# tanm-sys/forge-ec

Hardware: AMD Instinct MI355X
Metric: secp256k1-var scalar-muls/sec (batched, bit-exact vs CPU oracle on the parity sample) (higher is better)
Workload: dtype u32

## Files before the change

### forge_ec_amd/build.py

```python
import hashlib
import os
import subprocess
import sys

HERE = os.path.dirname(os.path.abspath(__file__))
SRC_DIR = os.path.join(HERE, "csrc")
OBJ_DIR = os.path.join(SRC_DIR, "_obj")
SO = os.path.join(HERE, "libfecgpu.so")
STAMP = SO + ".sha256"
SOURCES = ["fecgpu.hip", "canon.hip", "kernels_p256.hip", "kernels_ed.hip", "kernels_secp.hip", "kernels_codec.hip", "kernels_ecdsa.hip", "kernels_x25519.hip"]
HEADERS = ["coop.hpp", "sched_lf.hpp", "limbs.hpp", "staging.hpp", "host_ctx.hpp", "secp256k1.hpp", "p256.hpp", "ed25519.hpp", "curve25519.hpp",
           "canon_curves.hpp", "canon_kernels.hpp", "field_asm.inc", "kernels.hpp", "cu_split.hpp", os.path.join("..", "..", "include", "fecgpu.h"),
           os.path.join("..", "..", "include", "fecgpu_canon.h")]
FLAGS = ["--offload-arch=gfx950", "-O3", "-std=c++17", "-fPIC"]


def source_hash():
    h = hashlib.sha256(" ".join(FLAGS).encode())
    for rel in SOURCES + HEADERS:
        with open(os.path.join(SRC_DIR, rel), "rb") as f:
            h.update(rel.encode() + b"\0" + f.read())
    return h.hexdigest()


def up_to_date():
    try:
        return os.path.exists(SO) and open(STAMP).read().strip() == source_hash()
    except OSError:
        return False


DECLARATION_ONLY = ("kernels.hpp",)


def tu_closure_hash(src, kernel_code_only=False):
    import re
    seen, todo = [], [src]
    while todo:
        rel = todo.pop()
        if rel in seen or not os.path.exists(os.path.join(SRC_DIR, rel)) or (kernel_code_only and rel in DECLARATION_ONLY):
            continue
        seen.append(rel)
        with open(os.path.join(SRC_DIR, rel), "r") as f:
            todo += re.findall(r'^\s*#\s*include\s+"([^"/]+)"', f.read(), flags=re.M)
    h = hashlib.sha256(" ".join(FLAGS).encode())
    for rel in sorted(seen):
        with open(os.path.join(SRC_DIR, rel), "rb") as f:
            h.update(rel.encode() + b"\0" + f.read())
    return h.hexdigest()


WORKLOAD_TU = {"secp256k1-var": "kernels_secp.hip", "secp256k1-fixed": "kernels_secp.hip",
               "p256-var": "kernels_p256.hip", "p256-fixed": "kernels_p256.hip",
               "ed25519-var": "kernels_ed.hip", "ed25519-fixed": "kernels_ed.hip", "secp256k1-double": "kernels_secp.hip"}


def _tu_hash(src):
    return tu_closure_hash(src)


def build(force=False, verbose=False):
    if not force and up_to_date():
        return SO
    hipcc = os.environ.get("HIPCC", "/opt/rocm/bin/hipcc")
# ... 39 lines not shown
```

### forge_ec_amd/csrc/field_asm.inc

```
#pragma once

#define FEC_SECP_MUL_ASM \
      "v_mov_b32_e32 v165, 0\n\t" \
      "v_mov_b32_e32 v163, 0\n\t" \
      "v_mad_u64_u32 v[132:133], vcc, %10, %18, 0\n\t" \
      "v_mov_b32_e32 v162, v133\n\t" \
      "v_mad_u64_u32 v[134:135], vcc, %10, %19, v[162:163]\n\t" \
      "v_mad_u64_u32 v[134:135], vcc, %11, %18, v[134:135]\n\t" \
      "v_addc_co_u32_e32 v163, vcc, 0, v163, vcc\n\t" \
      "v_mul_lo_u32 v133, v132, %26\n\t" \
      "v_mov_b32_e32 v162, v135\n\t" \
      "v_mad_u64_u32 v[166:167], %9, v133, %27, 0\n\t" \
      "v_add_co_u32_e64 v164, %8, v167, v133\n\t" \
      "v_mad_u64_u32 v[136:137], vcc, %10, %20, v[162:163]\n\t" \
      "v_addc_co_u32_e64 v163, vcc, 0, 0, vcc\n\t" \
      "v_sub_u32_e32 v135, v134, v164\n\t" \
      "v_mad_u64_u32 v[136:137], vcc, %11, %19, v[136:137]\n\t" \
      "v_addc_co_u32_e32 v163, vcc, 0, v163, vcc\n\t" \
      "v_mul_lo_u32 v135, v135, %26\n\t" \
      "v_mad_u64_u32 v[136:137], vcc, %12, %18, v[136:137]\n\t" \
      "v_addc_co_u32_e32 v163, vcc, 0, v163, vcc\n\t" \
      "v_mad_u64_u32 v[166:167], %9, v135, %27, v[164:165]\n\t" \
      "v_mov_b32_e32 v162, v137\n\t" \
      "v_addc_co_u32_e64 v164, %8, v167, v135, %8\n\t" \
// ... 1235 lines not shown
      "v_alignbit_b32 v126, v126, v124, 31\n\t" \
      "v_lshlrev_b32_e32 v124, 1, v124\n\t" \
      "v_add_co_u32_e32 v124, vcc, v124, v153\n\t" \
      "v_addc_co_u32_e32 v126, vcc, v126, v154, vcc\n\t" \
      "v_addc_co_u32_e32 v128, vcc, v128, v155, vcc\n\t" \
      "v_addc_co_u32_e32 v130, vcc, v130, v156, vcc\n\t" \
      "v_addc_co_u32_e32 v132, vcc, v132, v157, vcc\n\t" \
      "v_addc_co_u32_e32 v134, vcc, v134, v158, vcc\n\t" \
      "v_addc_co_u32_e32 v136, vcc, v136, v159, vcc\n\t" \
      "v_addc_co_u32_e32 v138, vcc, v138, v160, vcc\n\t" \
      "v_addc_co_u32_e32 v140, vcc, v140, v161, vcc\n\t" \
      "v_addc_co_u32_e32 v142, vcc, v142, v162, vcc\n\t" \
      "v_addc_co_u32_e32 v144, vcc, v144, v163, vcc\n\t" \
      "v_addc_co_u32_e32 v146, vcc, v146, v164, vcc\n\t" \
      "v_addc_co_u32_e32 v148, vcc, v148, v165, vcc\n\t" \
      "v_addc_co_u32_e32 v149, vcc, v149, v166, vcc\n\t" \
      "v_addc_co_u32_e32 v151, vcc, v151, v167, vcc\n\t" \
      "v_mov_b32_e32 v153, 0\n\t" \
      "v_mov_b32_e32 v125, 0\n\t" \
      "v_mov_b32_e32 v127, 0\n\t" \
      "v_mov_b32_e32 v129, 0\n\t" \
      "v_mov_b32_e32 v131, 0\n\t" \
      "v_mov_b32_e32 v133, 0\n\t" \
      "v_mov_b32_e32 v135, 0\n\t" \
      "v_mov_b32_e32 v137, 0\n\t" \
      "v_mad_u64_u32 v[152:153], %8, v138, 38, v[152:153]\n\t" \
      "v_mad_u64_u32 v[124:125], %8, v140, 38, v[124:125]\n\t" \
      "v_mad_u64_u32 v[126:127], %8, v142, 38, v[126:127]\n\t" \
      "v_mad_u64_u32 v[128:129], %8, v144, 38, v[128:129]\n\t" \
      "v_mad_u64_u32 v[130:131], %8, v146, 38, v[130:131]\n\t" \
      "v_mad_u64_u32 v[132:133], %8, v148, 38, v[132:133]\n\t" \
      "v_mad_u64_u32 v[134:135], %8, v149, 38, v[134:135]\n\t" \
      "v_mad_u64_u32 v[136:137], %8, v151, 38, v[136:137]\n\t" \
      "v_add_co_u32_e32 %1, vcc, v124, v153\n\t" \
      "v_addc_co_u32_e32 %2, vcc, v126, v125, vcc\n\t" \
      "v_addc_co_u32_e32 %3, vcc, v128, v127, vcc\n\t" \
      "v_addc_co_u32_e32 %4, vcc, v130, v129, vcc\n\t" \
      "v_addc_co_u32_e32 %5, vcc, v132, v131, vcc\n\t" \
      "v_addc_co_u32_e32 %6, vcc, v134, v133, vcc\n\t" \
      "v_addc_co_u32_e32 %7, vcc, v136, v135, vcc\n\t" \
      "v_addc_co_u32_e32 v150, vcc, 0, v137, vcc\n\t" \
      "v_mul_u32_u24_e32 v150, 19, v150\n\t" \
      "v_add_co_u32_e32 %0, vcc, v152, v150\n\t" \
      "s_mov_b64 %9, vcc\n\t" \
      "v_lshrrev_b32_e32 v150, 31, %7\n\t" \
      "v_and_b32_e32 %7, 0x7fffffff, %7\n\t" \
      "v_mul_u32_u24_e32 v150, 19, v150\n\t" \
      "v_add_co_u32_e32 %0, vcc, %0, v150\n\t" \
      "s_or_b64 %9, %9, vcc\n\t" \
      "v_cmp_eq_u32_e32 vcc, 0x7fffffff, %7\n\t" \
      "s_or_b64 %9, %9, vcc"

#define FEC_ED_SQR_CLOBBERS "vcc", "v122", "v123", "v124", "v125", "v126", "v127", "v128", "v129", "v130", "v131", "v132", "v133", "v134", "v135", "v136", "v137", "v138", "v139", "v140", "v141", "v142", "v143", "v144", "v145", "v146", "v147", "v148", "v149", "v150", "v151", "v152", "v153", "v154", "v155", "v156", "v157", "v158", "v159", "v160", "v161", "v162", "v163", "v164", "v165", "v166", "v167"
```

### forge_ec_amd/csrc/kernels_secp.hip

```cpp
#include <hip/hip_runtime.h>

#include "../../include/fecgpu.h"
#include "secp256k1.hpp"
#include "staging.hpp"
#include "kernels.hpp"

namespace fecgpu {

namespace {

FEC_DEV secp::pt ld3(const u32* l, int stride) {
  secp::pt p;
  FEC_UNROLL for (int i = 0; i < 8; ++i) {
    p.x.w[i] = l[i * stride];
    p.y.w[i] = l[(8 + i) * stride];
    p.z.w[i] = l[(16 + i) * stride];
  }
  return p;
}
FEC_DEV void st3(u32* l, int stride, const secp::pt& p) {
  FEC_UNROLL for (int i = 0; i < 8; ++i) {
    l[i * stride] = p.x.w[i];
    l[(8 + i) * stride] = p.y.w[i];
    l[(16 + i) * stride] = p.z.w[i];
  }
}

FEC_DEV fe ldc(const u32* l, int c) {
  fe a;
  FEC_UNROLL for (int i = 0; i < 8; ++i) a.w[i] = l[(8 * c + i) * TPB];
  return a;
}

FEC_DEV secp::pt padd_slots(const u32* lp, const u32* lq, lmask& need_double) {
  using namespace secp;
  fe z1s, z1c, z2s, z2c;
  lmask maybe;
  {
    const fe z1 = ldc(lp, 2);
    maybe = lanes_where(z1.w[0] == 0u);
    z1s = sqr(z1);
    z1c = mul(z1s, z1);
  }
  __builtin_amdgcn_sched_barrier(0);
  {
    const fe z2 = ldc(lq, 2);
    maybe |= lanes_where(z2.w[0] == 0u);
    z2s = sqr(z2);
    z2c = mul(z2s, z2);
  }
  __builtin_amdgcn_sched_barrier(0);
  const fe u1 = mul(ldc(lp, 0), z2s);
  const fe u2 = mul(ldc(lq, 0), z1s);
  __builtin_amdgcn_sched_barrier(0);
  const fe s1 = mul(ldc(lp, 1), z2c);
  const fe s2 = mul(ldc(lq, 1), z1c);
// ... 28 lines not shown

template <int MODE>
__global__ __launch_bounds__(TPB, 3) void k_secp_mul(const u32* __restrict__ scalars,
                                                  const u32* __restrict__ points,
                                                  u32* __restrict__ out, size_t n,
                                                  const u32* __restrict__ prefix, int wbits) {
  __shared__ u32 lds[48 * TPB];
  const int valid = block_valid(n);
  const size_t first = (size_t)blockIdx.x * TPB;
  const int e = threadIdx.x;
  if (MODE == 0) stage_in<24>(lds, points + first * 24, valid);
  __syncthreads();
  if (e < valid) {
    const size_t g = first + e;
    const u32* kg = scalars + g * 8;
    lmask early = 0;
    u32* const slot0 = lds + e;
    int i0 = 0, i1 = 256;
    if (MODE != 3) {
      u32 any = 0;
      FEC_UNROLL for (int i = 0; i < 8; ++i) any |= kg[i];
      early = lanes_where(any == 0);
    }
    if (MODE == 2) early |= secp::is_identity(ld3(points, 1));
    if (MODE == 2 || MODE == 3) {
      const u32 idx = MODE == 3 ? (u32)(g >> 1) : __builtin_bswap32(kg[0]) >> (32 - wbits);
      const uint4* row = reinterpret_cast<const uint4*>(prefix + (size_t)idx * 48);
      FEC_UNROLL for (int q = 0; q < 12; ++q) {
        const uint4 x = row[q];
        slot0[(4 * q + 0) * TPB] = x.x;
        slot0[(4 * q + 1) * TPB] = x.y;
        slot0[(4 * q + 2) * TPB] = x.z;
        slot0[(4 * q + 3) * TPB] = x.w;
      }
      i0 = MODE == 3 ? 0 : wbits;
      if (MODE == 3) i1 = 1;
    } else {
      const secp::pt r1 = MODE != 0 ? ld3(points, 1) : ld3(lds + e, TPB);
      early |= secp::is_identity(r1);
      st3(slot0, TPB, secp::identity());
      st3(slot0 + 24 * TPB, TPB, r1);
    }
    u32 kword = MODE == 3 ? 0u : kg[i0 >> 5];
#pragma unroll 1
    for (int i = i0; i < i1; ++i) {
      u32 b;
      if (MODE == 3) {
        b = (u32)g & 1u;
      } else {
        if ((i & 31) == 0) kword = kg[i >> 5];
        const int sh = (((i >> 3) & 3) << 3) + 7 - (i & 7);
        b = (kword >> sh) & 1u;
      }
      lmask nd;
      secp::pt s = padd_slots(slot0, slot0 + 24 * TPB, nd);
      if (__builtin_expect(nd != 0, 0)) {
        secp::pt d0 = secp::pdouble(ld3(slot0, TPB));
        s = secp::pt_select(s, d0, nd);
      }
      u32* const slot_d = slot0 + b * (24u * TPB);
      u32* const slot_s = slot0 + (b ^ 1u) * (24u * TPB);
      const secp::pt din = ld3(slot_d, TPB);
      st3(slot_s, TPB, s);
      st3(slot_d, TPB, secp::pdouble(din));
    }
    if (MODE != 3) {
      const secp::pt r0 = secp::pt_select(ld3(slot0, TPB), secp::identity(), early);
      st3(slot0, TPB, r0);
    }
  }
  __syncthreads();
  if (MODE == 3) stage_out<48>(out + first * 48, lds, valid);
  else stage_out<24>(out + first * 24, lds, valid);
}

void secp_launch_mul(const SchedEnv& env, bool fixed, const u32* scalars, const u32* points, u32* out, size_t n, hipStream_t s) {
  const unsigned grid = (unsigned)((n + TPB - 1) / TPB);
  const int w = (int)env.gen_prefix_bits[FEC_SECP256K1];
  if (fixed && w > 0 && points == env.gen[FEC_SECP256K1] && env.gen_prefix[FEC_SECP256K1] != nullptr)
    hipLaunchKernelGGL((k_secp_mul<2>), dim3(grid), dim3(TPB), 0, s, scalars, points, out, n, env.gen_prefix[FEC_SECP256K1], w);
  else if (fixed) hipLaunchKernelGGL((k_secp_mul<1>), dim3(grid), dim3(TPB), 0, s, scalars, points, out, n, (const u32*)nullptr, 0);
  else hipLaunchKernelGGL((k_secp_mul<0>), dim3(grid), dim3(TPB), 0, s, scalars, points, out, n, (const u32*)nullptr, 0);
}

void secp_prefix_level_launch(const u32* parent, u32* child, size_t child_entries, hipStream_t s) {
  hipLaunchKernelGGL((k_secp_mul<3>), dim3((unsigned)((child_entries + TPB - 1) / TPB)), dim3(TPB), 0, s, (const u32*)nullptr,
                     (const u32*)nullptr, child, child_entries, parent, 0);
}

}
```

Baseline: 36.38 million.

## Add lazy-reduction secp ladder step with exact fallback on rare carries

New measurement: 37.14 million (median of 6 runs). 2.1% higher.

```diff
diff --git a/forge_ec_amd/build.py b/forge_ec_amd/build.py
--- a/forge_ec_amd/build.py
+++ b/forge_ec_amd/build.py
@@ -9,7 +9,7 @@
 SO = os.path.join(HERE, "libfecgpu.so")
 STAMP = SO + ".sha256"
 SOURCES = ["fecgpu.hip", "canon.hip", "kernels_p256.hip", "kernels_ed.hip", "kernels_secp.hip", "kernels_codec.hip", "kernels_ecdsa.hip", "kernels_x25519.hip"]
-HEADERS = ["coop.hpp", "sched_lf.hpp", "limbs.hpp", "staging.hpp", "host_ctx.hpp", "secp256k1.hpp", "p256.hpp", "ed25519.hpp", "curve25519.hpp",
+HEADERS = ["coop.hpp", "sched_lf.hpp", "limbs.hpp", "staging.hpp", "host_ctx.hpp", "secp256k1.hpp", "secp_step.hpp", "p256.hpp", "ed25519.hpp", "curve25519.hpp",
            "canon_curves.hpp", "canon_kernels.hpp", "field_asm.inc", "kernels.hpp", "cu_split.hpp", os.path.join("..", "..", "include", "fecgpu.h"),
            os.path.join("..", "..", "include", "fecgpu_canon.h")]
 FLAGS = ["--offload-arch=gfx950", "-O3", "-std=c++17", "-fPIC"]
diff --git a/forge_ec_amd/csrc/field_asm.inc b/forge_ec_amd/csrc/field_asm.inc
--- a/forge_ec_amd/csrc/field_asm.inc
+++ b/forge_ec_amd/csrc/field_asm.inc
@@ -1311,3 +1311,543 @@
       "s_or_b64 %9, %9, vcc"
 
 #define FEC_ED_SQR_CLOBBERS "vcc", "v122", "v123", "v124", "v125", "v126", "v127", "v128", "v129", "v130", "v131", "v132", "v133", "v134", "v135", "v136", "v137", "v138", "v139", "v140", "v141", "v142", "v143", "v144", "v145", "v146", "v147", "v148", "v149", "v150", "v151", "v152", "v153", "v154", "v155", "v156", "v157", "v158", "v159", "v160", "v161", "v162", "v163", "v164", "v165", "v166", "v167"
+
+
+#define FEC_SECP_MUL_ACC_ASM \
+      "v_mov_b32_e32 v165, 0\n\t" \
+      "v_mov_b32_e32 v163, 0\n\t" \
+      "v_mad_u64_u32 v[132:133], vcc, %11, %19, 0\n\t" \
+      "v_mov_b32_e32 v162, v133\n\t" \
+      "v_mad_u64_u32 v[134:135], vcc, %11, %20, v[162:163]\n\t" \
+      "v_mad_u64_u32 v[134:135], vcc, %12, %19, v[134:135]\n\t" \
+      "v_addc_co_u32_e32 v163, vcc, 0, v163, vcc\n\t" \
+      "v_mul_lo_u32 v133, v132, %27\n\t" \
+      "v_mov_b32_e32 v162, v135\n\t" \
+      "v_mad_u64_u32 v[166:167], %9, v133, %28, 0\n\t" \
+      "v_add_co_u32_e64 v164, %8, v167, v133\n\t" \
+      "v_mad_u64_u32 v[136:137], vcc, %11, %21, v[162:163]\n\t" \
+      "v_addc_co_u32_e64 v163, vcc, 0, 0, vcc\n\t" \
+      "v_sub_u32_e32 v135, v134, v164\n\t" \
+      "v_mad_u64_u32 v[136:137], vcc, %12, %20, v[136:137]\n\t" \
+      "v_addc_co_u32_e32 v163, vcc, 0, v163, vcc\n\t" \
+      "v_mul_lo_u32 v135, v135, %27\n\t" \
+      "v_mad_u64_u32 v[136:137], vcc, %13, %19, v[136:137]\n\t" \
+      "v_addc_co_u32_e32 v163, vcc, 0, v163, vcc\n\t" \
+      "v_mad_u64_u32 v[166:167], %9, v135, %28, v[164:165]\n\t" \
+      "v_mov_b32_e32 v162, v137\n\t" \
+      "v_addc_co_u32_e64 v164, %8, v167, v135, %8\n\t" \
+      "v_mad_u64_u32 v[138:139], vcc, %11, %22, v[162:163]\n\t" \
+      "v_addc_co_u32_e64 v163, vcc, 0, 0, vcc\n\t" \
+      "v_sub_u32_e32 v137, v136, v164\n\t" \
+      "v_mad_u64_u32 v[138:139], vcc, %12, %21, v[138:139]\n\t" \
+      "v_addc_co_u32_e32 v163, vcc, 0, v163, vcc\n\t" \
+      "v_mul_lo_u32 v137, v137, %27\n\t" \
+      "v_mad_u64_u32 v[138:139], vcc, %13, %20, v[138:139]\n\t" \
+      "v_addc_co_u32_e32 v163, vcc, 0, v163, vcc\n\t" \
+      "v_mad_u64_u32 v[166:167], %9, v137, %28, v[164:165]\n\t" \
+      "v_mad_u64_u32 v[138:139], vcc, %14, %19, v[138:139]\n\t" \
+      "v_addc_co_u32_e32 v163, vcc, 0, v163, vcc\n\t" \
+      "v_addc_co_u32_e64 v164, %8, v167, v137, %8\n\t" \
+      "v_mov_b32_e32 v162, v139\n\t" \
+      "v_mad_u64_u32 v[140:141], vcc, %11, %23, v[162:163]\n\t" \
+      "v_addc_co_u32_e64 v163, vcc, 0, 0, vcc\n\t" \
+      "v_sub_u32_e32 v139, v138, v164\n\t" \
+      "v_mad_u64_u32 v[140:141], vcc, %12, %22, v[140:141]\n\t" \
+      "v_addc_co_u32_e32 v163, vcc, 0, v163, vcc\n\t" \
+      "v_mul_lo_u32 v139, v139, %27\n\t" \
+      "v_mad_u64_u32 v[140:141], vcc, %13, %21, v[140:141]\n\t" \
+      "v_addc_co_u32_e32 v163, vcc, 0, v163, vcc\n\t" \
+      "v_mad_u64_u32 v[166:167], %9, v139, %28, v[164:165]\n\t" \
+      "v_mad_u64_u32 v[140:141], vcc, %14, %20, v[140:141]\n\t" \
+      "v_addc_co_u32_e32 v163, vcc, 0, v163, vcc\n\t" \
+      "v_addc_co_u32_e64 v164, %8, v167, v139, %8\n\t" \
+      "v_mad_u64_u32 v[140:141], vcc, %15, %19, v[140:141]\n\t" \
+      "v_addc_co_u32_e32 v163, vcc, 0, v163, vcc\n\t" \
+      "v_mov_b32_e32 v162, v141\n\t" \
+      "v_mad_u64_u32 v[142:143], vcc, %11, %24, v[162:163]\n\t" \
+      "v_addc_co_u32_e64 v163, vcc, 0, 0, vcc\n\t" \
+      "v_sub_u32_e32 v141, v140, v164\n\t" \
+      "v_mad_u64_u32 v[142:143], vcc, %12, %23, v[142:143]\n\t" \
+      "v_addc_co_u32_e32 v163, vcc, 0, v163, vcc\n\t" \
+      "v_mul_lo_u32 v141, v141, %27\n\t" \
+      "v_mad_u64_u32 v[142:143], vcc, %13, %22, v[142:143]\n\t" \
+      "v_addc_co_u32_e32 v163, vcc, 0, v163, vcc\n\t" \
+      "v_mad_u64_u32 v[166:167], %9, v141, %28, v[164:165]\n\t" \
+      "v_mad_u64_u32 v[142:143], vcc, %14, %21, v[142:143]\n\t" \
+      "v_addc_co_u32_e32 v163, vcc, 0, v163, vcc\n\t" \
+      "v_addc_co_u32_e64 v164, %8, v167, v141, %8\n\t" \
+      "v_mad_u64_u32 v[142:143], vcc, %15, %20, v[142:143]\n\t" \
+      "v_addc_co_u32_e32 v163, vcc, 0, v163, vcc\n\t" \
+      "v_mad_u64_u32 v[142:143], vcc, %16, %19, v[142:143]\n\t" \
+      "v_addc_co_u32_e32 v163, vcc, 0, v163, vcc\n\t" \
+      "v_mov_b32_e32 v162, v143\n\t" \
+      "v_mad_u64_u32 v[144:145], vcc, %11, %25, v[162:163]\n\t" \
+      "v_addc_co_u32_e64 v163, vcc, 0, 0, vcc\n\t" \
+      "v_sub_u32_e32 v143, v142, v164\n\t" \
+      "v_mad_u64_u32 v[144:145], vcc, %12, %24, v[144:145]\n\t" \
+      "v_addc_co_u32_e32 v163, vcc, 0, v163, vcc\n\t" \
+      "v_mul_lo_u32 v143, v143, %27\n\t" \
+      "v_mad_u64_u32 v[144:145], vcc, %13, %23, v[144:145]\n\t" \
+      "v_addc_co_u32_e32 v163, vcc, 0, v163, vcc\n\t" \
+      "v_mad_u64_u32 v[166:167], %9, v143, %28, v[164:165]\n\t" \
+      "v_mad_u64_u32 v[144:145], vcc, %14, %22, v[144:145]\n\t" \
+      "v_addc_co_u32_e32 v163, vcc, 0, v163, vcc\n\t" \
+      "v_addc_co_u32_e64 v164, %8, v167, v143, %8\n\t" \
+      "v_mad_u64_u32 v[144:145], vcc, %15, %21, v[144:145]\n\t" \
+      "v_addc_co_u32_e32 v163, vcc, 0, v163, vcc\n\t" \
+      "v_mad_u64_u32 v[144:145], vcc, %16, %20, v[144:145]\n\t" \
+      "v_addc_co_u32_e32 v163, vcc, 0, v163, vcc\n\t" \
+      "v_mad_u64_u32 v[144:145], vcc, %17, %19, v[144:145]\n\t" \
+      "v_addc_co_u32_e32 v163, vcc, 0, v163, vcc\n\t" \
+      "v_mov_b32_e32 v162, v145\n\t" \
+      "v_mad_u64_u32 v[146:147], vcc, %11, %26, v[162:163]\n\t" \
+      "v_addc_co_u32_e64 v163, vcc, 0, 0, vcc\n\t" \
+      "v_sub_u32_e32 v145, v144, v164\n\t" \
+      "v_mad_u64_u32 v[146:147], vcc, %12, %25, v[146:147]\n\t" \
+      "v_addc_co_u32_e32 v163, vcc, 0, v163, vcc\n\t" \
+      "v_mul_lo_u32 v145, v145, %27\n\t" \
+      "v_mad_u64_u32 v[146:147], vcc, %13, %24, v[146:147]\n\t" \
+      "v_addc_co_u32_e32 v163, vcc, 0, v163, vcc\n\t" \
+      "v_mad_u64_u32 v[166:167], %9, v145, %28, v[164:165]\n\t" \
+      "v_mad_u64_u32 v[146:147], vcc, %14, %23, v[146:147]\n\t" \
+      "v_addc_co_u32_e32 v163, vcc, 0, v163, vcc\n\t" \
+      "v_addc_co_u32_e64 v164, %8, v167, v145, %8\n\t" \
+      "v_mad_u64_u32 v[146:147], vcc, %15, %22, v[146:147]\n\t" \
+      "v_addc_co_u32_e32 v163, vcc, 0, v163, vcc\n\t" \
+      "v_mad_u64_u32 v[146:147], vcc, %16, %21, v[146:147]\n\t" \
+      "v_addc_co_u32_e32 v163, vcc, 0, v163, vcc\n\t" \
+      "v_mad_u64_u32 v[146:147], vcc, %17, %20, v[146:147]\n\t" \
+      "v_addc_co_u32_e32 v163, vcc, 0, v163, vcc\n\t" \
+      "v_mad_u64_u32 v[146:147], vcc, %18, %19, v[146:147]\n\t" \
+      "v_addc_co_u32_e32 v163, vcc, 0, v163, vcc\n\t" \
+      "v_mov_b32_e32 v162, v147\n\t" \
+      "v_mad_u64_u32 v[148:149], vcc, %12, %26, v[162:163]\n\t" \
+      "v_addc_co_u32_e64 v163, vcc, 0, 0, vcc\n\t" \
+      "v_sub_u32_e32 v147, v146, v164\n\t" \
+      "v_mad_u64_u32 v[148:149], vcc, %13, %25, v[148:149]\n\t" \
+      "v_addc_co_u32_e32 v163, vcc, 0, v163, vcc\n\t" \
+      "v_mul_lo_u32 v147, v147, %27\n\t" \
+      "v_mad_u64_u32 v[148:149], vcc, %14, %24, v[148:149]\n\t" \
+      "v_addc_co_u32_e32 v163, vcc, 0, v163, vcc\n\t" \
+      "v_mad_u64_u32 v[166:167], %9, v147, %28, v[164:165]\n\t" \
+      "v_mad_u64_u32 v[148:149], vcc, %15, %23, v[148:149]\n\t" \
+      "v_addc_co_u32_e32 v163, vcc, 0, v163, vcc\n\t" \
+      "v_addc_co_u32_e64 v164, %8, v167, v147, %8\n\t" \
+      "v_mad_u64_u32 v[148:149], vcc, %16, %22, v[148:149]\n\t" \
+      "v_addc_co_u32_e32 v163, vcc, 0, v163, vcc\n\t" \
+      "v_mad_u64_u32 v[148:149], vcc, %17, %21, v[148:149]\n\t" \
+      "v_addc_co_u32_e32 v163, vcc, 0, v163, vcc\n\t" \
+      "v_mad_u64_u32 v[148:149], vcc, %18, %20, v[148:149]\n\t" \
+      "v_addc_co_u32_e32 v163, vcc, 0, v163, vcc\n\t" \
+      "v_mov_b32_e32 v162, v149\n\t" \
+      "v_mad_u64_u32 v[150:151], vcc, %13, %26, v[162:163]\n\t" \
+      "v_addc_co_u32_e64 v163, vcc, 0, 0, vcc\n\t" \
+      "v_mad_u64_u32 v[150:151], vcc, %14, %25, v[150:151]\n\t" \
+      "v_addc_co_u32_e32 v163, vcc, 0, v163, vcc\n\t" \
+      "v_mad_u64_u32 v[150:151], vcc, %15, %24, v[150:151]\n\t" \
+      "v_addc_co_u32_e32 v163, vcc, 0, v163, vcc\n\t" \
+      "v_mad_u64_u32 v[150:151], vcc, %16, %23, v[150:151]\n\t" \
+      "v_addc_co_u32_e32 v163, vcc, 0, v163, vcc\n\t" \
+      "v_mad_u64_u32 v[150:151], vcc, %17, %22, v[150:151]\n\t" \
+      "v_addc_co_u32_e32 v163, vcc, 0, v163, vcc\n\t" \
+      "v_mad_u64_u32 v[150:151], vcc, %18, %21, v[150:151]\n\t" \
+      "v_addc_co_u32_e32 v163, vcc, 0, v163, vcc\n\t" \
+      "v_mov_b32_e32 v162, v151\n\t" \
+      "v_mad_u64_u32 v[152:153], vcc, %14, %26, v[162:163]\n\t" \
+      "v_addc_co_u32_e64 v163, vcc, 0, 0, vcc\n\t" \
+      "v_mad_u64_u32 v[152:153], vcc, %15, %25, v[152:153]\n\t" \
+      "v_addc_co_u32_e32 v163, vcc, 0, v163, vcc\n\t" \
+      "v_mad_u64_u32 v[152:153], vcc, %16, %24, v[152:153]\n\t" \
+      "v_addc_co_u32_e32 v163, vcc, 0, v163, vcc\n\t" \
+      "v_mad_u64_u32 v[152:153], vcc, %17, %23, v[152:153]\n\t" \
+      "v_addc_co_u32_e32 v163, vcc, 0, v163, vcc\n\t" \
+      "v_mad_u64_u32 v[152:153], vcc, %18, %22, v[152:153]\n\t" \
+      "v_addc_co_u32_e32 v163, vcc, 0, v163, vcc\n\t" \
+      "v_mov_b32_e32 v162, v153\n\t" \
+      "v_mad_u64_u32 v[154:155], vcc, %15, %26, v[162:163]\n\t" \
+      "v_addc_co_u32_e64 v163, vcc, 0, 0, vcc\n\t" \
+      "v_mad_u64_u32 v[154:155], vcc, %16, %25, v[154:155]\n\t" \
+      "v_addc_co_u32_e32 v163, vcc, 0, v163, vcc\n\t" \
+      "v_mad_u64_u32 v[154:155], vcc, %17, %24, v[154:155]\n\t" \
+      "v_addc_co_u32_e32 v163, vcc, 0, v163, vcc\n\t" \
+      "v_mad_u64_u32 v[154:155], vcc, %18, %23, v[154:155]\n\t" \
+      "v_addc_co_u32_e32 v163, vcc, 0, v163, vcc\n\t" \
+      "v_mov_b32_e32 v162, v155\n\t" \
+      "v_mad_u64_u32 v[156:157], vcc, %16, %26, v[162:163]\n\t" \
+      "v_addc_co_u32_e64 v163, vcc, 0, 0, vcc\n\t" \
+      "v_mad_u64_u32 v[156:157], vcc, %17, %25, v[156:157]\n\t" \
+      "v_addc_co_u32_e32 v163, vcc, 0, v163, vcc\n\t" \
+      "v_mad_u64_u32 v[156:157], vcc, %18, %24, v[156:157]\n\t" \
+      "v_addc_co_u32_e32 v163, vcc, 0, v163, vcc\n\t" \
+      "v_mov_b32_e32 v162, v157\n\t" \
+      "v_mad_u64_u32 v[158:159], vcc, %17, %26, v[162:163]\n\t" \
+      "v_addc_co_u32_e64 v163, vcc, 0, 0, vcc\n\t" \
+      "v_mad_u64_u32 v[158:159], vcc, %18, %25, v[158:159]\n\t" \
+      "v_addc_co_u32_e32 v163, vcc, 0, v163, vcc\n\t" \
+      "v_mov_b32_e32 v162, v159\n\t" \
+      "v_mad_u64_u32 v[160:161], vcc, %18, %26, v[162:163]\n\t" \
+      "v_add_co_u32_e32 %0, vcc, v148, v133\n\t" \
+      "v_addc_co_u32_e32 %1, vcc, v150, v135, vcc\n\t" \
+      "v_addc_co_u32_e32 %2, vcc, v152, v137, vcc\n\t" \
+      "v_addc_co_u32_e32 %3, vcc, v154, v139, vcc\n\t" \
+      "v_addc_co_u32_e32 %4, vcc, v156, v141, vcc\n\t" \
+      "v_addc_co_u32_e32 %5, vcc, v158, v143, vcc\n\t" \
+      "v_addc_co_u32_e32 %6, vcc, v160, v145, vcc\n\t" \
+      "v_addc_co_u32_e32 %7, vcc, v161, v147, vcc\n\t" \
+      "v_cndmask_b32_e64 v165, 0, 1, %8\n\t" \
+      "v_sub_co_u32_e32 %0, vcc, %0, v164\n\t" \
+      "v_subb_co_u32_e32 %1, vcc, %1, v165, vcc\n\t" \
+      "s_or_b64 %10, %10, vcc"
+
+#define FEC_SECP_MUL_ACC_CLOBBERS "vcc", "v132", "v133", "v134", "v135", "v136", "v137", "v138", "v139", "v140", "v141", "v142", "v143", "v144", "v145", "v146", "v147", "v148", "v149", "v150", "v151", "v152", "v153", "v154", "v155", "v156", "v157", "v158", "v159", "v160", "v161", "v162", "v163", "v164", "v165", "v166", "v167"
+
+
+#define FEC_SECP_SQR_ACC_ASM \
+      "v_mov_b32_e32 v135, 0\n\t" \
+      "v_mad_u64_u32 v[138:139], vcc, %10, %10, 0\n\t" \
+      "v_mov_b32_e32 v134, v139\n\t" \
+      "v_mad_u64_u32 v[140:141], vcc, %10, %11, v[134:135]\n\t" \
+      "v_mad_u64_u32 v[140:141], vcc, %11, %10, v[140:141]\n\t" \
+      "v_addc_co_u32_e64 v137, vcc, 0, 0, vcc\n\t" \
+      "v_mov_b32_e32 v136, v141\n\t" \
+      "v_mad_u64_u32 v[142:143], vcc, %11, %11, v[136:137]\n\t" \
+      "v_mad_u64_u32 v[144:145], vcc, %12, %12, 0\n\t" \
+      "v_mov_b32_e32 v134, v145\n\t" \
+      "v_mad_u64_u32 v[146:147], vcc, %12, %13, v[134:135]\n\t" \
+      "v_mad_u64_u32 v[146:147], vcc, %13, %12, v[146:147]\n\t" \
+      "v_addc_co_u32_e64 v137, vcc, 0, 0, vcc\n\t" \
+      "v_mov_b32_e32 v136, v147\n\t" \
+      "v_mad_u64_u32 v[148:149], vcc, %13, %13, v[136:137]\n\t" \
+      "v_mad_u64_u32 v[150:151], vcc, %14, %14, 0\n\t" \
+      "v_mov_b32_e32 v134, v151\n\t" \
+      "v_mad_u64_u32 v[152:153], vcc, %14, %15, v[134:135]\n\t" \
+      "v_mad_u64_u32 v[152:153], vcc, %15, %14, v[152:153]\n\t" \
+      "v_addc_co_u32_e64 v137, vcc, 0, 0, vcc\n\t" \
+      "v_mov_b32_e32 v136, v153\n\t" \
+      "v_mad_u64_u32 v[154:155], vcc, %15, %15, v[136:137]\n\t" \
+      "v_mad_u64_u32 v[156:157], vcc, %16, %16, 0\n\t" \
+      "v_mov_b32_e32 v134, v157\n\t" \
+      "v_mad_u64_u32 v[158:159], vcc, %16, %17, v[134:135]\n\t" \
+      "v_mad_u64_u32 v[158:159], vcc, %17, %16, v[158:159]\n\t" \
+      "v_addc_co_u32_e64 v137, vcc, 0, 0, vcc\n\t" \
+      "v_mov_b32_e32 v136, v159\n\t" \
+      "v_mad_u64_u32 v[160:161], vcc, %17, %17, v[136:137]\n\t" \
+      "v_mad_u64_u32 v[162:163], vcc, %10, %12, 0\n\t" \
+      "v_mov_b32_e32 v134, v163\n\t" \
+      "v_mad_u64_u32 v[164:165], vcc, %10, %13, v[134:135]\n\t" \
+      "v_mad_u64_u32 v[164:165], vcc, %11, %12, v[164:165]\n\t" \
+      "v_addc_co_u32_e64 v137, vcc, 0, 0, vcc\n\t" \
+      "v_mov_b32_e32 v136, v165\n\t" \
+      "v_mad_u64_u32 v[166:167], vcc, %11, %13, v[136:137]\n\t" \
+      "v_alignbit_b32 v167, v167, v166, 31\n\t" \
+      "v_alignbit_b32 v166, v166, v164, 31\n\t" \
+      "v_alignbit_b32 v164, v164, v162, 31\n\t" \
+      "v_lshlrev_b32_e32 v162, 1, v162\n\t" \
+      "v_add_co_u32_e32 v142, vcc, v142, v162\n\t" \
+      "v_addc_co_u32_e32 v143, vcc, v143, v164, vcc\n\t" \
+      "s_mov_b64 %8, vcc\n\t" \
+      "v_add_co_u32_e32 v144, vcc, v144, v166\n\t" \
+      "v_addc_co_u32_e32 v146, vcc, v146, v167, vcc\n\t" \
+      "s_or_b64 vcc, vcc, %8\n\t" \
+      "v_addc_co_u32_e32 v148, vcc, 0, v148, vcc\n\t" \
+      "v_addc_co_u32_e32 v149, vcc, 0, v149, vcc\n\t" \
+      "s_or_b64 %9, %9, vcc\n\t" \
+      "v_mad_u64_u32 v[162:163], vcc, %10, %14, 0\n\t" \
+      "v_mov_b32_e32 v134, v163\n\t" \
+      "v_mad_u64_u32 v[164:165], vcc, %10, %15, v[134:135]\n\t" \
+      "v_mad_u64_u32 v[164:165], vcc, %11, %14, v[164:165]\n\t" \
+      "v_addc_co_u32_e64 v137, vcc, 0, 0, vcc\n\t" \
+      "v_mov_b32_e32 v136, v165\n\t" \
+      "v_mad_u64_u32 v[166:167], vcc, %11, %15, v[136:137]\n\t" \
+      "v_alignbit_b32 v167, v167, v166, 31\n\t" \
+      "v_alignbit_b32 v166, v166, v164, 31\n\t" \
+      "v_alignbit_b32 v164, v164, v162, 31\n\t" \
+      "v_lshlrev_b32_e32 v162, 1, v162\n\t" \
+      "v_add_co_u32_e32 %4, vcc, v144, v162\n\t" \
+      "v_addc_co_u32_e32 %5, vcc, v146, v164, vcc\n\t" \
+      "s_mov_b64 %8, vcc\n\t" \
+      "v_add_co_u32_e32 v148, vcc, v148, v166\n\t" \
+      "v_addc_co_u32_e32 v149, vcc, v149, v167, vcc\n\t" \
+      "s_or_b64 vcc, vcc, %8\n\t" \
+      "v_addc_co_u32_e32 v150, vcc, 0, v150, vcc\n\t" \
+      "v_addc_co_u32_e32 v152, vcc, 0, v152, vcc\n\t" \
+      "s_or_b64 %9, %9, vcc\n\t" \
+      "v_mad_u64_u32 v[162:163], vcc, %10, %16, 0\n\t" \
+      "v_mov_b32_e32 v134, v163\n\t" \
+      "v_mad_u64_u32 v[164:165], vcc, %10, %17, v[134:135]\n\t" \
+      "v_mad_u64_u32 v[164:165], vcc, %11, %16, v[164:165]\n\t" \
+      "v_addc_co_u32_e64 v137, vcc, 0, 0, vcc\n\t" \
+      "v_mov_b32_e32 v136, v165\n\t" \
+      "v_mad_u64_u32 v[166:167], vcc, %11, %17, v[136:137]\n\t" \
+      "v_alignbit_b32 v167, v167, v166, 31\n\t" \
+      "v_alignbit_b32 v166, v166, v164, 31\n\t" \
+      "v_alignbit_b32 v164, v164, v162, 31\n\t" \
+      "v_lshlrev_b32_e32 v162, 1, v162\n\t" \
+      "v_add_co_u32_e32 v148, vcc, v148, v162\n\t" \
+      "v_addc_co_u32_e32 v149, vcc, v149, v164, vcc\n\t" \
+      "s_mov_b64 %8, vcc\n\t" \
+      "v_add_co_u32_e32 v150, vcc, v150, v166\n\t" \
+      "v_addc_co_u32_e32 v152, vcc, v152, v167, vcc\n\t" \
+      "s_or_b64 vcc, vcc, %8\n\t" \
+      "v_addc_co_u32_e32 v154, vcc, 0, v154, vcc\n\t" \
+      "v_addc_co_u32_e32 v155, vcc, 0, v155, vcc\n\t" \
+      "s_or_b64 %9, %9, vcc\n\t" \
+      "v_mad_u64_u32 v[162:163], vcc, %12, %14, 0\n\t" \
+      "v_mov_b32_e32 v134, v163\n\t" \
+      "v_mad_u64_u32 v[164:165], vcc, %12, %15, v[134:135]\n\t" \
+      "v_mad_u64_u32 v[164:165], vcc, %13, %14, v[164:165]\n\t" \
+      "v_addc_co_u32_e64 v137, vcc, 0, 0, vcc\n\t" \
+      "v_mov_b32_e32 v136, v165\n\t" \
+      "v_mad_u64_u32 v[166:167], vcc, %13, %15, v[136:137]\n\t" \
+      "v_alignbit_b32 v167, v167, v166, 31\n\t" \
+      "v_alignbit_b32 v166, v166, v164, 31\n\t" \
+      "v_alignbit_b32 v164, v164, v162, 31\n\t" \
+      "v_lshlrev_b32_e32 v162, 1, v162\n\t" \
+      "v_add_co_u32_e32 %6, vcc, v148, v162\n\t" \
+      "v_addc_co_u32_e32 %7, vcc, v149, v164, vcc\n\t" \
+      "s_mov_b64 %8, vcc\n\t" \
+      "v_add_co_u32_e32 v150, vcc, v150, v166\n\t" \
+      "v_addc_co_u32_e32 v152, vcc, v152, v167, vcc\n\t" \
+      "s_or_b64 vcc, vcc, %8\n\t" \
+      "v_addc_co_u32_e32 v154, vcc, 0, v154, vcc\n\t" \
+      "v_addc_co_u32_e32 v155, vcc, 0, v155, vcc\n\t" \
+      "s_or_b64 %9, %9, vcc\n\t" \
+      "v_mad_u64_u32 v[162:163], vcc, %12, %16, 0\n\t" \
+      "v_mov_b32_e32 v134, v163\n\t" \
+      "v_mad_u64_u32 v[164:165], vcc, %12, %17, v[134:135]\n\t" \
+      "v_mad_u64_u32 v[164:165], vcc, %13, %16, v[164:165]\n\t" \
+      "v_addc_co_u32_e64 v137, vcc, 0, 0, vcc\n\t" \
+      "v_mov_b32_e32 v136, v165\n\t" \
+      "v_mad_u64_u32 v[166:167], vcc, %13, %17, v[136:137]\n\t" \
+      "v_alignbit_b32 v167, v167, v166, 31\n\t" \
+      "v_alignbit_b32 v166, v166, v164, 31\n\t" \
+      "v_alignbit_b32 v164, v164, v162, 31\n\t" \
+      "v_lshlrev_b32_e32 v162, 1, v162\n\t" \
+      "v_add_co_u32_e32 v150, vcc, v150, v162\n\t" \
+      "v_addc_co_u32_e32 v152, vcc, v152, v164, vcc\n\t" \
+      "s_mov_b64 %8, vcc\n\t" \
+      "v_add_co_u32_e32 v154, vcc, v154, v166\n\t" \
+      "v_addc_co_u32_e32 v155, vcc, v155, v167, vcc\n\t" \
+      "s_or_b64 vcc, vcc, %8\n\t" \
+      "v_addc_co_u32_e32 v156, vcc, 0, v156, vcc\n\t" \
+      "v_addc_co_u32_e32 v158, vcc, 0, v158, vcc\n\t" \
+      "s_or_b64 %9, %9, vcc\n\t" \
+      "v_mad_u64_u32 v[162:163], vcc, %14, %16, 0\n\t" \
+      "v_mov_b32_e32 v134, v163\n\t" \
+      "v_mad_u64_u32 v[164:165], vcc, %14, %17, v[134:135]\n\t" \
+      "v_mad_u64_u32 v[164:165], vcc, %15, %16, v[164:165]\n\t" \
+      "v_addc_co_u32_e64 v137, vcc, 0, 0, vcc\n\t" \
+      "v_mov_b32_e32 v136, v165\n\t" \
+      "v_mad_u64_u32 v[166:167], vcc, %15, %17, v[136:137]\n\t" \
+      "v_alignbit_b32 v167, v167, v166, 31\n\t" \
+      "v_alignbit_b32 v166, v166, v164, 31\n\t" \
+      "v_alignbit_b32 v164, v164, v162, 31\n\t" \
+      "v_lshlrev_b32_e32 v162, 1, v162\n\t" \
+      "v_add_co_u32_e32 v154, vcc, v154, v162\n\t" \
+      "v_addc_co_u32_e32 v155, vcc, v155, v164, vcc\n\t" \
+      "s_mov_b64 %8, vcc\n\t" \
+      "v_add_co_u32_e32 v156, vcc, v156, v166\n\t" \
+      "v_addc_co_u32_e32 v158, vcc, v158, v167, vcc\n\t" \
+      "s_or_b64 vcc, vcc, %8\n\t" \
+      "v_addc_co_u32_e32 v160, vcc, 0, v160, vcc\n\t" \
+      "v_addc_co_u32_e32 v161, vcc, 0, v161, vcc\n\t" \
+      "v_mad_u64_u32 v[162:163], vcc, v150, %18, 0\n\t" \
+      "v_mul_lo_u32 v164, v152, %18\n\t" \
+      "v_add3_u32 v164, v163, v164, v150\n\t" \
+      "v_add_co_u32_e32 v138, vcc, v138, v162\n\t" \
+      "v_addc_co_u32_e32 v140, vcc, v140, v164, vcc\n\t" \
+      "v_addc_co_u32_e32 v142, vcc, 0, v142, vcc\n\t" \
+      "v_addc_co_u32_e32 v143, vcc, 0, v143, vcc\n\t" \
+      "s_or_b64 %9, %9, vcc\n\t" \
+      "v_mad_u64_u32 v[162:163], vcc, v154, %18, 0\n\t" \
+      "v_mul_lo_u32 v164, v155, %18\n\t" \
+      "v_add3_u32 v164, v163, v164, v154\n\t" \
+      "v_add_co_u32_e32 v138, vcc, v138, v162\n\t" \
+      "v_addc_co_u32_e32 v140, vcc, v140, v164, vcc\n\t" \
+      "v_addc_co_u32_e32 v142, vcc, 0, v142, vcc\n\t" \
+      "v_addc_co_u32_e32 v143, vcc, 0, v143, vcc\n\t" \
+      "s_or_b64 %9, %9, vcc\n\t" \
+      "v_mad_u64_u32 v[162:163], vcc, v156, %18, 0\n\t" \
+      "v_mul_lo_u32 v164, v158, %18\n\t" \
+      "v_add3_u32 v164, v163, v164, v156\n\t" \
+      "v_add_co_u32_e32 v138, vcc, v138, v162\n\t" \
+      "v_addc_co_u32_e32 v140, vcc, v140, v164, vcc\n\t" \
+      "v_addc_co_u32_e32 v142, vcc, 0, v142, vcc\n\t" \
+      "v_addc_co_u32_e32 v143, vcc, 0, v143, vcc\n\t" \
+      "s_or_b64 %9, %9, vcc\n\t" \
+      "v_mad_u64_u32 v[162:163], vcc, v160, %18, 0\n\t" \
+      "v_mul_lo_u32 v164, v161, %18\n\t" \
+      "v_add3_u32 v164, v163, v164, v160\n\t" \
+      "v_add_co_u32_e32 %0, vcc, v138, v162\n\t" \
+      "v_addc_co_u32_e32 %1, vcc, v140, v164, vcc\n\t" \
+      "v_addc_co_u32_e32 %2, vcc, 0, v142, vcc\n\t" \
+      "v_addc_co_u32_e32 %3, vcc, 0, v143, vcc\n\t" \
+      "s_or_b64 %9, %9, vcc"
+
+#define FEC_SECP_SQR_ACC_CLOBBERS "vcc", "v134", "v135", "v136", "v137", "v138", "v139", "v140", "v141", "v142", "v143", "v144", "v145", "v146", "v147", "v148", "v149", "v150", "v151", "v152", "v153", "v154", "v155", "v156", "v157", "v158", "v159", "v160", "v161", "v162", "v163", "v164", "v165", "v166", "v167"
+
+
+#define FEC_SECP_MUL3_ACC_ASM \
+      "v_mov_b32_e32 v163, 0\n\t" \
+      "v_mov_b32_e32 v165, 0\n\t" \
+      "v_mad_u64_u32 v[146:147], %9, %11, 3, 0\n\t" \
+      "v_mov_b32_e32 v162, v147\n\t" \
+      "v_mad_u64_u32 v[148:149], %9, %12, 3, v[162:163]\n\t" \
+      "v_mov_b32_e32 v162, v149\n\t" \
+      "v_mad_u64_u32 v[150:151], %9, %13, 3, v[162:163]\n\t" \
+      "v_mov_b32_e32 v162, v151\n\t" \
+      "v_mad_u64_u32 v[152:153], %9, %14, 3, v[162:163]\n\t" \
+      "v_mov_b32_e32 v162, v153\n\t" \
+      "v_mad_u64_u32 v[154:155], %9, %15, 3, v[162:163]\n\t" \
+      "v_mov_b32_e32 v162, v155\n\t" \
+      "v_mad_u64_u32 v[156:157], %9, %16, 3, v[162:163]\n\t" \
+      "v_mov_b32_e32 v162, v157\n\t" \
+      "v_mad_u64_u32 v[158:159], %9, %17, 3, v[162:163]\n\t" \
+      "v_mov_b32_e32 v162, v159\n\t" \
+      "v_mad_u64_u32 v[160:161], %9, %18, 3, v[162:163]\n\t" \
+      "v_mul_lo_u32 %0, v146, %19\n\t" \
+      "v_mad_u64_u32 v[166:167], %9, %0, %20, 0\n\t" \
+      "v_add_co_u32_e64 v164, %8, v167, %0\n\t" \
+      "v_sub_u32_e32 %1, v148, v164\n\t" \
+      "v_mul_lo_u32 %1, %1, %19\n\t" \
+      "v_mad_u64_u32 v[166:167], %9, %1, %20, v[164:165]\n\t" \
+      "v_addc_co_u32_e64 v164, %8, v167, %1, %8\n\t" \
+      "v_sub_u32_e32 %2, v150, v164\n\t" \
+      "v_mul_lo_u32 %2, %2, %19\n\t" \
+      "v_mad_u64_u32 v[166:167], %9, %2, %20, v[164:165]\n\t" \
+      "v_addc_co_u32_e64 v164, %8, v167, %2, %8\n\t" \
+      "v_sub_u32_e32 %3, v152, v164\n\t" \
+      "v_mul_lo_u32 %3, %3, %19\n\t" \
+      "v_mad_u64_u32 v[166:167], %9, %3, %20, v[164:165]\n\t" \
+      "v_addc_co_u32_e64 v164, %8, v167, %3, %8\n\t" \
+      "v_sub_u32_e32 %4, v154, v164\n\t" \
+      "v_mul_lo_u32 %4, %4, %19\n\t" \
+      "v_mad_u64_u32 v[166:167], %9, %4, %20, v[164:165]\n\t" \
+      "v_addc_co_u32_e64 v164, %8, v167, %4, %8\n\t" \
+      "v_sub_u32_e32 %5, v156, v164\n\t" \
+      "v_mul_lo_u32 %5, %5, %19\n\t" \
+      "v_mad_u64_u32 v[166:167], %9, %5, %20, v[164:165]\n\t" \
+      "v_addc_co_u32_e64 v164, %8, v167, %5, %8\n\t" \
+      "v_sub_u32_e32 %6, v158, v164\n\t" \
+      "v_mul_lo_u32 %6, %6, %19\n\t" \
+      "v_mad_u64_u32 v[166:167], %9, %6, %20, v[164:165]\n\t" \
+      "v_addc_co_u32_e64 v164, %8, v167, %6, %8\n\t" \
+      "v_sub_u32_e32 %7, v160, v164\n\t" \
+      "v_mul_lo_u32 %7, %7, %19\n\t" \
+      "v_mad_u64_u32 v[166:167], %9, %7, %20, v[164:165]\n\t" \
+      "v_addc_co_u32_e64 v164, %8, v167, %7, %8\n\t" \
+      "v_add_co_u32_e32 %0, vcc, %0, v161\n\t" \
+      "s_or_b64 %10, %10, vcc\n\t" \
+      "v_cndmask_b32_e64 v165, 0, 1, %8\n\t" \
+      "v_sub_co_u32_e32 %0, vcc, %0, v164\n\t" \
+      "v_subb_co_u32_e32 %1, vcc, %1, v165, vcc\n\t" \
+      "s_or_b64 %10, %10, vcc"
+
+#define FEC_SECP_MUL3_ACC_CLOBBERS "vcc", "v146", "v147", "v148", "v149", "v150", "v151", "v152", "v153", "v154", "v155", "v156", "v157", "v158", "v159", "v160", "v161", "v162", "v163", "v164", "v165", "v166", "v167"
+
+
+#define FEC_SECP_MUL8_ACC_ASM \
+      "v_mov_b32_e32 v163, 0\n\t" \
+      "v_mov_b32_e32 v165, 0\n\t" \
+      "v_mad_u64_u32 v[146:147], %9, %11, 8, 0\n\t" \
+      "v_mov_b32_e32 v162, v147\n\t" \
+      "v_mad_u64_u32 v[148:149], %9, %12, 8, v[162:163]\n\t" \
+      "v_mov_b32_e32 v162, v149\n\t" \
+      "v_mad_u64_u32 v[150:151], %9, %13, 8, v[162:163]\n\t" \
+      "v_mov_b32_e32 v162, v151\n\t" \
+      "v_mad_u64_u32 v[152:153], %9, %14, 8, v[162:163]\n\t" \
+      "v_mov_b32_e32 v162, v153\n\t" \
+      "v_mad_u64_u32 v[154:155], %9, %15, 8, v[162:163]\n\t" \
+      "v_mov_b32_e32 v162, v155\n\t" \
+      "v_mad_u64_u32 v[156:157], %9, %16, 8, v[162:163]\n\t" \
+      "v_mov_b32_e32 v162, v157\n\t" \
+      "v_mad_u64_u32 v[158:159], %9, %17, 8, v[162:163]\n\t" \
+      "v_mov_b32_e32 v162, v159\n\t" \
+      "v_mad_u64_u32 v[160:161], %9, %18, 8, v[162:163]\n\t" \
+      "v_mul_lo_u32 %0, v146, %19\n\t" \
+      "v_mad_u64_u32 v[166:167], %9, %0, %20, 0\n\t" \
+      "v_add_co_u32_e64 v164, %8, v167, %0\n\t" \
+      "v_sub_u32_e32 %1, v148, v164\n\t" \
+      "v_mul_lo_u32 %1, %1, %19\n\t" \
+      "v_mad_u64_u32 v[166:167], %9, %1, %20, v[164:165]\n\t" \
+      "v_addc_co_u32_e64 v164, %8, v167, %1, %8\n\t" \
+      "v_sub_u32_e32 %2, v150, v164\n\t" \
+      "v_mul_lo_u32 %2, %2, %19\n\t" \
+      "v_mad_u64_u32 v[166:167], %9, %2, %20, v[164:165]\n\t" \
+      "v_addc_co_u32_e64 v164, %8, v167, %2, %8\n\t" \
+      "v_sub_u32_e32 %3, v152, v164\n\t" \
+      "v_mul_lo_u32 %3, %3, %19\n\t" \
+      "v_mad_u64_u32 v[166:167], %9, %3, %20, v[164:165]\n\t" \
+      "v_addc_co_u32_e64 v164, %8, v167, %3, %8\n\t" \
+      "v_sub_u32_e32 %4, v154, v164\n\t" \
+      "v_mul_lo_u32 %4, %4, %19\n\t" \
+      "v_mad_u64_u32 v[166:167], %9, %4, %20, v[164:165]\n\t" \
+      "v_addc_co_u32_e64 v164, %8, v167, %4, %8\n\t" \
+      "v_sub_u32_e32 %5, v156, v164\n\t" \
+      "v_mul_lo_u32 %5, %5, %19\n\t" \
+      "v_mad_u64_u32 v[166:167], %9, %5, %20, v[164:165]\n\t" \
+      "v_addc_co_u32_e64 v164, %8, v167, %5, %8\n\t" \
+      "v_sub_u32_e32 %6, v158, v164\n\t" \
+      "v_mul_lo_u32 %6, %6, %19\n\t" \
+      "v_mad_u64_u32 v[166:167], %9, %6, %20, v[164:165]\n\t" \
+      "v_addc_co_u32_e64 v164, %8, v167, %6, %8\n\t" \
+      "v_sub_u32_e32 %7, v160, v164\n\t" \
+      "v_mul_lo_u32 %7, %7, %19\n\t" \
+      "v_mad_u64_u32 v[166:167], %9, %7, %20, v[164:165]\n\t" \
+      "v_addc_co_u32_e64 v164, %8, v167, %7, %8\n\t" \
+      "v_add_co_u32_e32 %0, vcc, %0, v161\n\t" \
+      "s_or_b64 %10, %10, vcc\n\t" \
+      "v_cndmask_b32_e64 v165, 0, 1, %8\n\t" \
+      "v_sub_co_u32_e32 %0, vcc, %0, v164\n\t" \
+      "v_subb_co_u32_e32 %1, vcc, %1, v165, vcc\n\t" \
+      "s_or_b64 %10, %10, vcc"
+
+#define FEC_SECP_MUL8_ACC_CLOBBERS "vcc", "v146", "v147", "v148", "v149", "v150", "v151", "v152", "v153", "v154", "v155", "v156", "v157", "v158", "v159", "v160", "v161", "v162", "v163", "v164", "v165", "v166", "v167"
+
+
+#define FEC_SECP_ADD_ACC_ASM \
+      "v_add_co_u32_e32 %0, vcc, %0, %11\n\t" \
+      "v_addc_co_u32_e32 %1, vcc, %1, %12, vcc\n\t" \
+      "v_addc_co_u32_e32 %2, vcc, %2, %13, vcc\n\t" \
+      "v_addc_co_u32_e32 %3, vcc, %3, %14, vcc\n\t" \
+      "v_addc_co_u32_e32 %4, vcc, %4, %15, vcc\n\t" \
+      "v_addc_co_u32_e32 %5, vcc, %5, %16, vcc\n\t" \
+      "v_addc_co_u32_e32 %6, vcc, %6, %17, vcc\n\t" \
+      "v_addc_co_u32_e32 %7, vcc, %7, %18, vcc\n\t" \
+      "v_cndmask_b32_e64 %9, 0, 1, vcc\n\t" \
+      "v_mul_u32_u24_e32 %10, 0x3d1, %9\n\t" \
+      "v_add_co_u32_e32 %0, vcc, %0, %10\n\t" \
+      "v_addc_co_u32_e32 %1, vcc, %1, %9, vcc\n\t" \
+      "s_or_b64 %8, %8, vcc"
+
+
+#define FEC_SECP_DBL_ACC_ASM \
+      "v_add_co_u32_e32 %0, vcc, %0, %0\n\t" \
+      "v_addc_co_u32_e32 %1, vcc, %1, %1, vcc\n\t" \
+      "v_addc_co_u32_e32 %2, vcc, %2, %2, vcc\n\t" \
+      "v_addc_co_u32_e32 %3, vcc, %3, %3, vcc\n\t" \
+      "v_addc_co_u32_e32 %4, vcc, %4, %4, vcc\n\t" \
+      "v_addc_co_u32_e32 %5, vcc, %5, %5, vcc\n\t" \
+      "v_addc_co_u32_e32 %6, vcc, %6, %6, vcc\n\t" \
+      "v_addc_co_u32_e32 %7, vcc, %7, %7, vcc\n\t" \
+      "v_cndmask_b32_e64 %9, 0, 1, vcc\n\t" \
+      "v_mul_u32_u24_e32 %10, 0x3d1, %9\n\t" \
+      "v_add_co_u32_e32 %0, vcc, %0, %10\n\t" \
+      "v_addc_co_u32_e32 %1, vcc, %1, %9, vcc\n\t" \
+      "s_or_b64 %8, %8, vcc"
+
+
+#define FEC_SECP_SUB_ACC_ASM \
+      "v_sub_co_u32_e32 %0, vcc, %0, %11\n\t" \
+      "v_subb_co_u32_e32 %1, vcc, %1, %12, vcc\n\t" \
+      "v_subb_co_u32_e32 %2, vcc, %2, %13, vcc\n\t" \
+      "v_subb_co_u32_e32 %3, vcc, %3, %14, vcc\n\t" \
+      "v_subb_co_u32_e32 %4, vcc, %4, %15, vcc\n\t" \
+      "v_subb_co_u32_e32 %5, vcc, %5, %16, vcc\n\t" \
+      "v_subb_co_u32_e32 %6, vcc, %6, %17, vcc\n\t" \
+      "v_subb_co_u32_e32 %7, vcc, %7, %18, vcc\n\t" \
+      "v_cndmask_b32_e64 %9, 0, 1, vcc\n\t" \
+      "v_mul_u32_u24_e32 %10, 0x3d1, %9\n\t" \
+      "v_sub_co_u32_e32 %0, vcc, %0, %10\n\t" \
+      "v_subb_co_u32_e32 %1, vcc, %1, %9, vcc\n\t" \
+      "s_or_b64 %8, %8, vcc"
diff --git a/forge_ec_amd/csrc/kernels_secp.hip b/forge_ec_amd/csrc/kernels_secp.hip
--- a/forge_ec_amd/csrc/kernels_secp.hip
+++ b/forge_ec_amd/csrc/kernels_secp.hip
@@ -2,6 +2,7 @@
 
 #include "../../include/fecgpu.h"
 #include "secp256k1.hpp"
+#include "secp_step.hpp"
 #include "staging.hpp"
 #include "kernels.hpp"
 
@@ -136,17 +137,18 @@
         const int sh = (((i >> 3) & 3) << 3) + 7 - (i & 7);
         b = (kword >> sh) & 1u;
       }
-      lmask nd;
-      secp::pt s = padd_slots(slot0, slot0 + 24 * TPB, nd);
-      if (__builtin_expect(nd != 0, 0)) {
-        secp::pt d0 = secp::pdouble(ld3(slot0, TPB));
-        s = secp::pt_select(s, d0, nd);
-      }
       u32* const slot_d = slot0 + b * (24u * TPB);
       u32* const slot_s = slot0 + (b ^ 1u) * (24u * TPB);
-      const secp::pt din = ld3(slot_d, TPB);
-      st3(slot_s, TPB, s);
-      st3(slot_d, TPB, secp::pdouble(din));
+      secp_step::add_step(slot0, slot0 + 24 * TPB, slot_s, [&]() {
+        lmask nd;
+        secp::pt s = padd_slots(slot0, slot0 + 24 * TPB, nd);
+        if (__builtin_expect(nd != 0, 0)) {
+          secp::pt d0 = secp::pdouble(ld3(slot0, TPB));
+          s = secp::pt_select(s, d0, nd);
+        }
+        return s;
+      });
+      secp_step::double_step(slot_d, [&]() { return secp::pdouble(ld3(slot_d, TPB)); });
     }
     if (MODE != 3) {
       const secp::pt r0 = secp::pt_select(ld3(slot0, TPB), secp::identity(), early);
diff --git a/forge_ec_amd/csrc/secp_step.hpp b/forge_ec_amd/csrc/secp_step.hpp
--- /dev/null
+++ b/forge_ec_amd/csrc/secp_step.hpp
@@ -0,0 +1,166 @@
+#pragma once
+#include "secp256k1.hpp"
+#include "staging.hpp"
+
+namespace fecgpu {
+namespace secp_step {
+
+using secp::pt;
+
+struct Rare {
+  lmask m = 0;
+  u32 top = 0;
+};
+FEC_DEV void note_top(Rare& rr, const fe& r) { rr.top = rr.top > r.w[7] ? rr.top : r.w[7]; }
+FEC_DEV bool met(const Rare& rr) { return (rr.m | lanes_where(rr.top == 0xFFFFFFFFu)) != 0; }
+
+FEC_DEV fe mul(const fe& a, const fe& b, Rare& rr) {
+  fe r;
+  lmask sc, sink;
+  asm(FEC_SECP_MUL_ACC_ASM
+      : "=v"(r.w[0]), "=v"(r.w[1]), "=v"(r.w[2]), "=v"(r.w[3]), "=v"(r.w[4]), "=v"(r.w[5]), "=v"(r.w[6]),
+        "=v"(r.w[7]), "=&s"(sc), "=&s"(sink), "+s"(rr.m)
+      : FEC_V8(a), FEC_V8(b), "s"(0xD2253531u), "s"(977u)
+      : FEC_SECP_MUL_ACC_CLOBBERS);
+  note_top(rr, r);
+  return r;
+}
+template <u32 K>
+FEC_DEV fe mul_small(const fe& a, Rare& rr) {
+  static_assert(K == 3 || K == 8, "the ladder multiplies by 3 and 8 only");
+  fe r;
+  lmask sc, sink;
+  if (K == 3) {
+    asm(FEC_SECP_MUL3_ACC_ASM
+        : "=v"(r.w[0]), "=v"(r.w[1]), "=v"(r.w[2]), "=v"(r.w[3]), "=v"(r.w[4]), "=v"(r.w[5]), "=v"(r.w[6]),
+          "=v"(r.w[7]), "=&s"(sc), "=&s"(sink), "+s"(rr.m)
+        : FEC_V8(a), "s"(0xD2253531u), "s"(977u)
+        : FEC_SECP_MUL3_ACC_CLOBBERS);
+  } else {
+    asm(FEC_SECP_MUL8_ACC_ASM
+        : "=v"(r.w[0]), "=v"(r.w[1]), "=v"(r.w[2]), "=v"(r.w[3]), "=v"(r.w[4]), "=v"(r.w[5]), "=v"(r.w[6]),
+          "=v"(r.w[7]), "=&s"(sc), "=&s"(sink), "+s"(rr.m)
+        : FEC_V8(a), "s"(0xD2253531u), "s"(977u)
+        : FEC_SECP_MUL8_ACC_CLOBBERS);
+  }
+  note_top(rr, r);
+  return r;
+}
+FEC_DEV fe sqr(const fe& a, Rare& rr) {
+  fe r;
+  lmask tmp;
+  asm(FEC_SECP_SQR_ACC_ASM
+      : "=v"(r.w[0]), "=v"(r.w[1]), "=v"(r.w[2]), "=v"(r.w[3]), "=&v"(r.w[4]), "=&v"(r.w[5]), "=&v"(r.w[6]),
+        "=&v"(r.w[7]), "=&s"(tmp), "+s"(rr.m)
+      : FEC_V8(a), "s"(977u)
+      : FEC_SECP_SQR_ACC_CLOBBERS);
+  note_top(rr, r);
+  return r;
+}
+FEC_DEV fe add(const fe& a, const fe& b, Rare& rr) {
+  fe x = a;
+  u32 t0, t1;
+  asm(FEC_SECP_ADD_ACC_ASM : FEC_RW8(x), "+s"(rr.m), "=&v"(t1), "=&v"(t0) : FEC_V8(b) : "vcc");
+  note_top(rr, x);
+  return x;
+}
+FEC_DEV fe dbl(const fe& a, Rare& rr) {
+  fe x = a;
+  u32 t0, t1;
+  asm(FEC_SECP_DBL_ACC_ASM : FEC_RW8(x), "+s"(rr.m), "=&v"(t1), "=&v"(t0) : : "vcc");
+  note_top(rr, x);
+  return x;
+}
+FEC_DEV fe sub(const fe& a, const fe& b, Rare& rr) {
+  fe x = a;
+  u32 t0, t1;
+  asm(FEC_SECP_SUB_ACC_ASM : FEC_RW8(x), "+s"(rr.m), "=&v"(t1), "=&v"(t0) : FEC_V8(b) : "vcc");
+  return x;
+}
+
+FEC_DEV fe ld(const u32* l, int c) {
+  fe a;
+  FEC_UNROLL for (int i = 0; i < 8; ++i) a.w[i] = l[(8 * c + i) * TPB];
+  return a;
+}
+FEC_DEV void st(u32* l, const pt& p) {
+  FEC_UNROLL for (int i = 0; i < 8; ++i) {
+    l[i * TPB] = p.x.w[i];
+    l[(8 + i) * TPB] = p.y.w[i];
+    l[(16 + i) * TPB] = p.z.w[i];
+  }
+}
+
+FEC_DEV void in_registers(const fe& a, u32 b) { asm volatile("" : : FEC_V8(a), "v"(b)); }
+FEC_DEV void in_registers(const fe& a, const fe& b) { asm volatile("" : : FEC_V8(a), FEC_V8(b)); }
+
+FEC_DEV bool padd_fast(const u32* lp, const u32* lq, pt& o) {
+  const fe z1 = ld(lp, 2);
+  const u32 z2w0 = lq[16 * TPB];
+  in_registers(z1, z2w0);
+  if (__builtin_expect(lanes_where((z1.w[0] < z2w0 ? z1.w[0] : z2w0) == 0u) != 0, 0)) return false;
+  Rare rr;
+  fe z1s, z1c, z2s, z2c;
+  {
+    z1s = sqr(z1, rr);
+    z1c = mul(z1s, z1, rr);
+  }
+  __builtin_amdgcn_sched_barrier(0);
+  {
+    const fe z2 = ld(lq, 2);
+    z2s = sqr(z2, rr);
+    z2c = mul(z2s, z2, rr);
+  }
+  __builtin_amdgcn_sched_barrier(0);
+  const fe u1 = mul(ld(lp, 0), z2s, rr);
+  const fe u2 = mul(ld(lq, 0), z1s, rr);
+  __builtin_amdgcn_sched_barrier(0);
+  const fe s1 = mul(ld(lp, 1), z2c, rr);
+  const fe s2 = mul(ld(lq, 1), z1c, rr);
+  __builtin_amdgcn_sched_barrier(0);
+  rr.m |= lanes_where(u1.w[0] == u2.w[0]);
+  const fe h = sub(u2, u1, rr);
+  const fe r = sub(s2, s1, rr);
+  const fe h2 = sqr(h, rr);
+  const fe h3 = mul(h2, h, rr);
+  const fe u1h2 = mul(u1, h2, rr);
+  o.x = sub(sub(sub(sqr(r, rr), h3, rr), u1h2, rr), u1h2, rr);
+  o.y = sub(mul(r, sub(u1h2, o.x, rr), rr), mul(s1, h3, rr), rr);
+  o.z = mul(mul(h, ld(lp, 2), rr), ld(lq, 2), rr);
+  return !met(rr);
+}
+
+FEC_DEV bool pdouble_fast(const u32* l, pt& r) {
+  const pt p = {ld(l, 0), ld(l, 1), ld(l, 2)};
+  in_registers(p.x, p.y);
+  in_registers(p.z, 0u);
+  if (__builtin_expect(lanes_where(p.z.w[0] == 0u) != 0, 0)) return false;
+  Rare rr;
+  const fe a = sqr(p.x, rr);
+  const fe b = sqr(p.y, rr);
+  const fe c = sqr(b, rr);
+  const fe xpb2 = sqr(add(p.x, b, rr), rr);
+  const fe d = dbl(sub(sub(xpb2, a, rr), c, rr), rr);
+  const fe e = mul_small<3>(a, rr);
+  const fe f = sqr(e, rr);
+  r.x = sub(f, dbl(d, rr), rr);
+  r.y = sub(mul(e, sub(d, r.x, rr), rr), mul_small<8>(c, rr), rr);
+  r.z = dbl(mul(p.y, p.z, rr), rr);
+  return !met(rr);
+}
+
+template <class Exact>
+FEC_DEV void add_step(const u32* lp, const u32* lq, u32* dst, Exact exact) {
+  pt o;
+  if (__builtin_expect(!padd_fast(lp, lq, o), 0)) o = exact();
+  st(dst, o);
+}
+template <class Exact>
+FEC_DEV void double_step(u32* l, Exact exact) {
+  pt o;
+  if (__builtin_expect(!pdouble_fast(l, o), 0)) o = exact();
+  st(l, o);
+}
+
+}
+}
```
